# FofanovLab/mtsv_tools

Measured on NVIDIA B200. Metric: reads/sec binned (150 bp), higher is better.
Workload: dtype u8/u32 integer

## Files before the change

### mtsv_tools_b200/csrc/binner.cu

```cuda
#include <algorithm>
#include <thread>

#include "ctx.h"

#ifndef MTSV_COALESCE_UNROLL
#define MTSV_COALESCE_UNROLL 4
#endif
#ifndef MTSV_COALESCE_TILES
#define MTSV_COALESCE_TILES 4
#endif
constexpr int kCoalesceTiles = MTSV_COALESCE_TILES;
constexpr int kCoalesceUnroll = MTSV_COALESCE_UNROLL;

namespace mtsv {

constexpr uint32_t kMaxReadLenDev = MTSVGPU_MAX_READ_LEN;

__device__ __forceinline__ void cta_accumulate(unsigned long long* counters32, unsigned int v) {
  __shared__ unsigned int cta_sum;
  if (threadIdx.x == 0) cta_sum = 0;
  __syncthreads();
  unsigned int w = __reduce_add_sync(0xffffffffu, v);
  if ((threadIdx.x & 31) == 0 && w) atomicAdd(&cta_sum, w);
  __syncthreads();
// ... 232 lines not shown
    unsigned big = __ballot_sync(0xffffffffu, cnt > kSolo);
    while (big) {
      int src = __ffs(big) - 1;
      big &= big - 1;
      uint32_t c = __shfl_sync(0xffffffffu, cnt, src);
      uint32_t l = __shfl_sync(0xffffffffu, lo, src);
      uint32_t d = __shfl_sync(0xffffffffu, dst, src);
      for (uint32_t r = lane; r < c; r += 32)
        hit_keys[d + r] = make_hit_key(fm_locate(fm, sv, l + r, nullptr), qoff);
    }
  }
}

constexpr uint32_t kSortMedium = 4096;
constexpr uint32_t kLightItems = 16;
constexpr uint32_t kMonsterHits = 1024;

__device__ __forceinline__ uint64_t warp_sort_u64(uint64_t v, unsigned lane) {
#pragma unroll
  for (int k = 2; k <= 32; k <<= 1) {
    {
      uint64_t o = __shfl_xor_sync(0xffffffffu, v, k - 1);
      bool low = (lane & (k - 1)) < ((lane ^ (k - 1)) & (k - 1));
      v = low ? (v < o ? v : o) : (v > o ? v : o);
    }
#pragma unroll
    for (int j = k >> 2; j > 0; j >>= 1) {
      uint64_t o = __shfl_xor_sync(0xffffffffu, v, j);
      bool low = (lane & j) == 0;
      v = low ? (v < o ? v : o) : (v > o ? v : o);
    }
  }
  return v;
}

__global__ void __launch_bounds__(256) sort_classify_kernel(const uint32_t* __restrict__ seg_cnt, uint32_t nq,
                                                            uint32_t min_count, uint32_t* __restrict__ warp_list,
                                                            uint32_t* __restrict__ medium_list,
                                                            uint32_t* __restrict__ large_list,
                                                            BatchCounters* __restrict__ ctr) {
  uint32_t q = blockIdx.x * blockDim.x + threadIdx.x;
  const unsigned lane = threadIdx.x & 31;
  uint32_t n = q < nq ? seg_cnt[q] : 0;
  int cls = n <= min_count || n < 2 ? -1 : (n <= 32 ? 0 : (n <= kSortMedium ? 1 : 2));
#pragma unroll
  for (int c = 0; c < 3; ++c) {
    unsigned m = __ballot_sync(0xffffffffu, cls == c);
    if (!m) continue;
    unsigned int* counter = c == 0 ? &ctr->n_warp : (c == 1 ? &ctr->n_medium : &ctr->n_large);
    uint32_t* list = c == 0 ? warp_list : (c == 1 ? medium_list : large_list);
    uint32_t base = 0;
    if (lane == (unsigned)(__ffs(m) - 1)) base = atomicAdd(counter, (unsigned)__popc(m));
    base = __shfl_sync(0xffffffffu, base, __ffs(m) - 1);
    if (cls == c) list[base + __popc(m & ((1u << lane) - 1))] = q;
  }
}

__global__ void __launch_bounds__(256) sort_warp_kernel(uint64_t* __restrict__ keys,
                                                        const uint32_t* __restrict__ seg_off,
                                                        const uint32_t* __restrict__ seg_cnt,
                                                        const uint32_t* __restrict__ list,
                                                        const BatchCounters* __restrict__ ctr) {
  const unsigned lane = threadIdx.x & 31;
  const uint32_t n_list = ctr->n_warp;
  const uint32_t warps = (gridDim.x * blockDim.x) >> 5;
  for (uint32_t it = (blockIdx.x * blockDim.x + threadIdx.x) >> 5; it < n_list; it += warps) {
    uint32_t q = list[it];
    uint32_t n = seg_cnt[q];
    uint64_t* base = keys + seg_off[q];
    uint64_t v = lane < n ? base[lane] : ~0ull;
// ... 100 lines not shown
  CE(0, 1) CE(2, 3) CE(4, 5) CE(6, 7) CE(8, 9) CE(10, 11) CE(12, 13) CE(14, 15)
  CE(0, 2) CE(1, 3) CE(4, 6) CE(5, 7) CE(8, 10) CE(9, 11) CE(12, 14) CE(13, 15)
  CE(1, 2) CE(5, 6) CE(9, 10) CE(13, 14) CE(0, 4) CE(1, 5) CE(2, 6) CE(3, 7)
  CE(8, 12) CE(9, 13) CE(10, 14) CE(11, 15) CE(2, 4) CE(3, 5) CE(10, 12) CE(11, 13)
  CE(1, 2) CE(3, 4) CE(5, 6) CE(9, 10) CE(11, 12) CE(13, 14) CE(0, 8) CE(1, 9)
  CE(2, 10) CE(3, 11) CE(4, 12) CE(5, 13) CE(6, 14) CE(7, 15) CE(4, 8) CE(5, 9)
  CE(6, 10) CE(7, 11) CE(2, 4) CE(3, 5) CE(6, 8) CE(7, 9) CE(10, 12) CE(11, 13)
  CE(1, 2) CE(3, 4) CE(5, 6) CE(7, 8) CE(9, 10) CE(11, 12) CE(13, 14)
#undef CE
}

__device__ __forceinline__ bool carry_valid_or_lane(unsigned lane, bool carry_valid) {
  return lane > 0 || carry_valid;
}

__device__ uint32_t coalesce_warp(const BinsView& bv, const uint64_t* __restrict__ keys, uint32_t n_hits,
                                  uint32_t min_seeds, uint32_t L, uint32_t k, CandRec* __restrict__ cand) {
  const unsigned lane = threadIdx.x & 31;
  uint32_t nc = 0;
  bool have = false;
  CandRec cur{0, 0, 0, 0};
  uint32_t carry_site = 0, carry_bin = 0;
  bool carry_valid = false;
  constexpr int U = kCoalesceTiles;
  uint32_t top = 1;
  while (top < bv.n) top <<= 1;
  for (uint32_t g0 = 0; g0 < n_hits; g0 += 32 * U) {
    uint32_t site[U], qoff[U], b[U], ws[U], we[U];
    bool some[U];
#pragma unroll
    for (int u = 0; u < U; ++u) {
      uint32_t h = g0 + u * 32 + lane;
      uint64_t key = h < n_hits ? keys[h] : 0;
      site[u] = (uint32_t)(key >> 16);
      qoff[u] = (uint32_t)(key & 0xffff);
      b[u] = 0;
    }
    for (uint32_t step = top; step >= 1; step >>= 1) {
#pragma unroll
// ... 75 lines not shown
          have = some_i;
          if (some_i) cur = CandRec{ws_i, we_i, b_i, 1};
        }
      }
    }
  }
  if (have && cur.num_seeds >= min_seeds) {
    if (lane == 0) {
      cand[nc] = cur;
    }
    ++nc;
  }
  return nc;
}

__global__ void __launch_bounds__(128) coalesce_kernel(BinsView bv, ReadsView rv, Params p, uint32_t nq,
                                                       const uint32_t* __restrict__ hit_off,
                                                       const uint32_t* __restrict__ q_nhits,
                                                       const uint32_t* __restrict__ q_nseeds,
                                                       uint64_t* __restrict__ hit_keys,
                                                       CandRec* __restrict__ cand_sparse,
                                                       uint32_t* __restrict__ q_ncand,
                                                       uint32_t* __restrict__ heavy_list,
                                                       uint32_t* __restrict__ monster_list,
                                                       BatchCounters* __restrict__ ctr) {
  const uint32_t r = blockIdx.x * blockDim.x + threadIdx.x;
  const unsigned lane = threadIdx.x & 31;
  uint32_t first = 0;
  if (p.ns == 2 && r * 2 + 1 < nq && q_nhits[r * 2 + 1] > q_nhits[r * 2]) first = 1;
  for (uint32_t pass = 0; pass < p.ns; ++pass) {
    const uint32_t s = p.ns == 2 ? (pass ^ first) : 0;
    const uint32_t q = r * p.ns + s;
    uint32_t nh = q < nq ? q_nhits[q] : 0;
    if (pass == 1 && !__any_sync(0xffffffffu, nh != 0)) {
      if (q < nq) q_ncand[q] = 0;
      continue;
    }
    uint32_t nc = 0, L = 0, k = 0, ms = 0, base = 0;
    if (nh) {
      L = query_len(rv, p.ns, q);
      k = edit_budget(L, p.edit_rate);
      ms = min_seeds_of(q_nseeds[q], p.min_seed);
      base = hit_off[q];
      if (nh <= kLightItems) {
        uint64_t* kq = hit_keys + base;
        if (nh > 1) {
          uint64_t v[kLightItems];
#pragma unroll
          for (uint32_t i = 0; i < kLightItems; ++i) v[i] = i < nh ? kq[i] : ~0ull;
          static_assert(kLightItems == 16, "sort_network16 sorts exactly 16 keys");
          sort_network16(v);
#pragma unroll
          for (uint32_t i = 0; i < kLightItems; ++i)
            if (i < nh) kq[i] = v[i];
        }
        nc = coalesce_item(bv, kq, nh, ms, L, k, cand_sparse + base);
      }
    }
    unsigned heavy = __ballot_sync(0xffffffffu, nh > kLightItems && nh <= kMonsterHits);
    if (heavy) {
      uint32_t slot = 0;
      if (lane == (unsigned)(__ffs(heavy) - 1)) slot = atomicAdd(&ctr->n_heavy, (unsigned)__popc(heavy));
      slot = __shfl_sync(0xffffffffu, slot, __ffs(heavy) - 1);
      if (nh > kLightItems && nh <= kMonsterHits) heavy_list[slot + __popc(heavy & ((1u << lane) - 1))] = q;
    }
    if (nh > kMonsterHits) monster_list[atomicAdd(&ctr->n_monster, 1u)] = q;
    if (q < nq && nh <= kLightItems) q_ncand[q] = nc;
  }
}

__global__ void __launch_bounds__(128) coalesce_heavy_kernel(BinsView bv, ReadsView rv, Params p,
                                                             const uint32_t* __restrict__ hit_off,
                                                             const uint32_t* __restrict__ q_nhits,
                                                             const uint32_t* __restrict__ q_nseeds,
                                                             const uint64_t* __restrict__ hit_keys,
                                                             CandRec* __restrict__ cand_sparse,
                                                             uint32_t* __restrict__ q_ncand,
                                                             const uint32_t* __restrict__ heavy_list,
                                                             BatchCounters* __restrict__ ctr) {
  const unsigned lane = threadIdx.x & 31;
  const uint32_t n_list = ctr->n_heavy;
  for (;;) {
// ... 63 lines not shown
      uint32_t run = 0;
      for (int i = 0; i < 32; ++i) {
        s_pre[i] = run;
        run += s_cnt[i];
      }
      s_pre[32] = run;
      q_ncand[q] = run;
    }
    __syncthreads();
    for (uint32_t i = lane; i < cnt; i += 32) cand_sparse[base + s_pre[w] + i] = cand_stage[base + my_start + i];
    __syncthreads();
  }
}

__global__ void __launch_bounds__(256) rank_emit_kernel(uint32_t nq, const uint32_t* __restrict__ hit_off,
                                                        const uint32_t* __restrict__ q_ncand,
                                                        const uint32_t* __restrict__ cand_off,
                                                        const CandRec* __restrict__ cand_sparse,
                                                        CandRec* __restrict__ cand_dense,
                                                        uint32_t* __restrict__ cand_q) {
  uint32_t q = blockIdx.x * blockDim.x + threadIdx.x;
  const unsigned lane = threadIdx.x & 31;
  uint32_t nc = q < nq ? q_ncand[q] : 0;
  uint32_t src = 0, dst = 0;
  if (nc) {
    src = hit_off[q];
    dst = cand_off[q];
    if (nc <= kLightItems) {
      uint64_t prev = 0;
      for (uint32_t i = 0; i < nc; ++i) {
        uint64_t best = ~0ull;
        for (uint32_t j = 0; j < nc; ++j) {
          uint64_t kj = make_rank_key(cand_sparse[src + j].num_seeds, j);
          if ((i == 0 || kj > prev) && kj < best) best = kj;
        }
        prev = best;
        cand_dense[dst + i] = cand_sparse[src + (uint32_t)(best & 0xffffffffu)];
        cand_q[dst + i] = q;
      }
    }
  }
  unsigned heavy = __ballot_sync(0xffffffffu, nc > kLightItems);
  while (heavy) {
    int sl = __ffs(heavy) - 1;
    heavy &= heavy - 1;
    const uint32_t nc_s = __shfl_sync(0xffffffffu, nc, sl), src_s = __shfl_sync(0xffffffffu, src, sl);
    const uint32_t dst_s = __shfl_sync(0xffffffffu, dst, sl), q_s = __shfl_sync(0xffffffffu, q, sl);
    uint32_t out = 0;
    uint32_t bound = 0xffffffffu;
    while (out < nc_s) {
      uint32_t v = 0;
      for (uint32_t i = lane; i < nc_s; i += 32) {
        uint32_t ns = cand_sparse[src_s + i].num_seeds;
        if (ns < bound && ns > v) v = ns;
      }
      v = __reduce_max_sync(0xffffffffu, v);
      for (uint32_t t0 = 0; t0 < nc_s; t0 += 32) {
// ... 625 lines not shown
    return set_error(MTSVGPU_EINVAL, "seed_size must be in [1,4096]");
  if (in->seed_gap == 0)
    return set_error(MTSVGPU_EINVAL, "seed_gap must be > 0");
  p->edit_rate = in->edit_rate;
  p->min_seed = in->min_seed;
  p->S = in->seed_size;
  p->G = in->seed_gap;
  p->max_hits = in->max_hits;
  p->tune_max_hits = in->tune_max_hits;
  p->max_candidates = in->max_candidates < 0 ? -1 : in->max_candidates;
  p->max_assignments = in->max_assignments < 0 ? -1 : in->max_assignments;
  p->ns = in->strands == 1 ? 1 : 2;
  return 0;
}

int run_segmented_sort(cudaStream_t st, DevBuf& worklist, uint64_t* keys, const uint32_t* seg_off,
                              const uint32_t* seg_cnt, uint32_t nq, uint32_t min_count, BatchCounters* d_ctr) {
  if (worklist.cap < (size_t)3 * nq * 4) {
    MTSV_CUDA_TRY(cudaStreamSynchronize(st));
    MTSV_TRY(worklist.reserve((size_t)3 * nq * 4));
  }
  uint32_t* lists = worklist.as<uint32_t>();
  MTSV_CUDA_TRY(cudaMemsetAsync(&d_ctr->n_warp, 0, 3 * sizeof(unsigned int), st));
  MTSV_LAUNCH(sort_classify_kernel, (nq + 255) / 256, 256, 0, st, seg_cnt, nq, min_count, lists, lists + nq,
              lists + 2 * (size_t)nq, d_ctr);
  MTSV_LAUNCH(sort_warp_kernel, sm_count() * 8, 256, 0, st, keys, seg_off, seg_cnt, lists, d_ctr);
  MTSV_LAUNCH(sort_medium_kernel, sm_count() * 4, 512, 0, st, keys, seg_off, seg_cnt, lists + nq, d_ctr);
  MTSV_LAUNCH(sort_large_kernel, sm_count(), 1024, 0, st, keys, seg_off, seg_cnt, lists + 2 * (size_t)nq, d_ctr);
  MTSV_CUDA_TRY(cudaGetLastError());
  return 0;
}

static int grow_preserve(DevBuf& buf, size_t used_bytes, size_t need_bytes, cudaStream_t st) {
  if (need_bytes <= buf.cap && buf.p) return 0;
  size_t want = std::max(need_bytes + need_bytes / 2, (size_t)1 << 20);
  DevPtr<uint8_t> np;
  MTSV_TRY(dev_alloc(np, want));
  if (buf.p && used_bytes) {
    MTSV_CUDA_TRY(cudaMemcpyAsync(np.get(), buf.p.get(), used_bytes, cudaMemcpyDeviceToDevice, st));
    MTSV_CUDA_TRY(cudaStreamSynchronize(st));
  }
  buf.p = std::move(np);
  buf.cap = want;
// ... 201 lines not shown
    if (rv.n_reads == 1)
      return set_error(MTSVGPU_ELIMIT, "one read produced %llu seed hits (cap %llu)", hc.total_hits,
                       (unsigned long long)hit_cap);
    return 1;
  }
  n_hits = (uint32_t)hc.total_hits;
  ln.stats.n_seed_hits += n_hits;
  for (int i = 0; i < 32; ++i) ln.stats.rank_queries += hc.rank_steps[i];
  return 0;
}

int SubBatch::candidates() {
  const DeviceIndex& ix = h->ix;
  for (DevBuf* b : {&ws.q_ncand, &ws.cand_off}) MTSV_TRY(b->reserve(qn * 4));
  if (!n_hits) return 0;
  MTSV_TRY(ws.worklist.reserve(3 * qn * 4));
  MTSV_TRY(ws.hit_keys.reserve((size_t)n_hits * 8));
  MTSV_TRY(ws.cand_sparse.reserve((size_t)n_hits * sizeof(CandRec)));
  begin(ST_LOCATE);
  MTSV_LAUNCH(locate_kernel, qgrid(), 256, 0, st, ix.fm_view(), ix.sa_view(), p, ws.slot_off.as<uint32_t>(), nq,
              ws.slot_lo.as<uint32_t>(), ws.slot_cnt.as<uint32_t>(), ws.slot_hoff.as<uint32_t>(),
              ws.hit_off.as<uint32_t>(), ws.q_nhits.as<uint32_t>(), ws.hit_keys.as<uint64_t>());
  end();
  begin(ST_SORT);
  MTSV_TRY(run_segmented_sort(st, ws.worklist, ws.hit_keys.as<uint64_t>(), ws.hit_off.as<uint32_t>(),
                              ws.q_nhits.as<uint32_t>(), nq, kLightItems, d_ctr));
  end();
  begin(ST_COALESCE);
  MTSV_TRY(ws.cand_stage.reserve((size_t)n_hits * sizeof(CandRec)));
  MTSV_CUDA_TRY(cudaMemsetAsync(&d_ctr->n_heavy, 0, 3 * sizeof(unsigned int), st));
  MTSV_LAUNCH(coalesce_kernel, (rv.n_reads + 127) / 128, 128, 0, st, ix.bins_view(), rv, p, nq,
              ws.hit_off.as<uint32_t>(), ws.q_nhits.as<uint32_t>(), ws.q_nseeds.as<uint32_t>(),
              ws.hit_keys.as<uint64_t>(), ws.cand_sparse.as<CandRec>(), ws.q_ncand.as<uint32_t>(),
              ws.worklist.as<uint32_t>(), ws.worklist.as<uint32_t>() + nq, d_ctr);
  MTSV_LAUNCH(coalesce_heavy_kernel, sm_count() * 16, 128, 0, st, ix.bins_view(), rv, p, ws.hit_off.as<uint32_t>(),
              ws.q_nhits.as<uint32_t>(), ws.q_nseeds.as<uint32_t>(), ws.hit_keys.as<uint64_t>(),
              ws.cand_sparse.as<CandRec>(), ws.q_ncand.as<uint32_t>(), ws.worklist.as<uint32_t>(), d_ctr);
  MTSV_LAUNCH(coalesce_monster_kernel, sm_count(), 1024, 0, st, ix.bins_view(), rv, p, ws.hit_off.as<uint32_t>(),
              ws.q_nhits.as<uint32_t>(), ws.q_nseeds.as<uint32_t>(), ws.hit_keys.as<uint64_t>(),
              ws.cand_sparse.as<CandRec>(), ws.cand_stage.as<CandRec>(), ws.q_ncand.as<uint32_t>(),
              ws.worklist.as<uint32_t>() + nq, d_ctr);
  MTSV_TRY(exclusive_scan_u32(ws.q_ncand.as<uint32_t>(), ws.cand_off.as<uint32_t>(), nq, ws.scan_tmp,
                              (uint64_t*)&d_ctr->total_cands, st));
  end();
  MTSV_TRY(fetch());
  n_cand = (uint32_t)hc.total_cands;
  if (!n_cand) return 0;
  MTSV_TRY(ws.cand_dense.reserve((size_t)n_cand * sizeof(CandRec)));
  MTSV_TRY(ws.cand_q.reserve((size_t)n_cand * 4));
  begin(ST_RANK);
  MTSV_LAUNCH(rank_emit_kernel, qgrid(), 256, 0, st, nq, ws.hit_off.as<uint32_t>(), ws.q_ncand.as<uint32_t>(),
              ws.cand_off.as<uint32_t>(), ws.cand_sparse.as<CandRec>(), ws.cand_dense.as<CandRec>(),
              ws.cand_q.as<uint32_t>());
  end();
  return 0;
}

int SubBatch::verify() {
  const bool ssw = hc.max_len >= 254;
  bool grouped = !ssw && (group_verify ? group_verify[0] != '0' : n_cand > nq && h->ix.n_bins > h->ix.n_taxids);
  MTSV_TRY(ws.cand_edit.reserve((size_t)n_cand * 4));
  begin(ST_VERIFY);
  MTSV_TRY(ws.cand_flag.reserve(((size_t)n_cand + 1) * 4));
  MTSV_TRY(ws.cand_order.reserve((size_t)n_cand * 4));
  MTSV_LAUNCH(cand_class_kernel, (n_cand + 255) / 256, 256, 0, st, ws.cand_dense.as<CandRec>(), n_cand,
              ws.cand_flag.as<uint32_t>(), (h->profiling && !grouped) ? d_ctr : nullptr, 1);
  MTSV_TRY(exclusive_scan_u32(ws.cand_flag.as<uint32_t>(), ws.cand_flag.as<uint32_t>(), n_cand, ws.scan_tmp,
                              nullptr, st));
// ... 79 lines not shown
  if (n2) {
    MTSV_LAUNCH(cand_compact_order_kernel, grid, 256, 0, st, ws.cand_order.as<uint32_t>(), flag, n_cand,
                ws.cand_dense.as<CandRec>(), ws.cand_order2.as<uint32_t>(), ctr);
    round_jobs.n = n2;
    MTSV_TRY(launch_verify_warp(round_jobs));
  }
  n_verified = (uint64_t)n1 + n2;
  return 0;
}

int SubBatch::merge_taxids() {
  const uint32_t nr = rv.n_reads;
  uint64_t* keys = ws.hit_keys.as<uint64_t>();
  MTSV_LAUNCH(taxid_keys_kernel, (nq + 1 + 255) / 256, 256, 0, st, nq, p.ns, ws.cand_off.as<uint32_t>(),
              ws.out_off.as<uint32_t>(), ws.hit_tmp.as<HitRec>(), keys, seg_off(), seg_cnt());
  MTSV_TRY(run_segmented_sort(st, ws.worklist, keys, seg_off(), seg_cnt(), nr, 1, d_ctr));
  MTSV_LAUNCH(taxid_count_kernel, (nr + 255) / 256, 256, 0, st, keys, seg_off(), nr, tax_cnt());
  MTSV_TRY(exclusive_scan_u32(tax_cnt(), tax_off(), nr, ws.scan_tmp, (uint64_t*)&d_ctr->total_taxhits, st));
  return 0;
}

int SubBatch::select_append(uint64_t* out_total) {
  for (DevBuf* b : {&ws.q_nout, &ws.out_off}) MTSV_TRY(b->reserve(qn * 4));
  const bool taxhits = kind == BatchOutput::TaxHits;
  uint64_t sub_out = 0, sub_tax = 0;
  if (n_cand) {
    MTSV_TRY(ws.hit_tmp.reserve((size_t)n_cand * sizeof(HitRec)));
    begin(ST_EMIT);
    MTSV_LAUNCH(select_kernel, (nq + 127) / 128, 128, 0, st, h->ix.bins_view(), rv, p, nq, ws.cand_off.as<uint32_t>(),
                ws.cand_dense.as<CandRec>(), ws.cand_edit.as<uint32_t>(), ws.hit_tmp.as<HitRec>(),
                ws.q_nout.as<uint32_t>());
// ... 313 lines not shown
```

### mtsv_tools_b200/csrc/collapse.cu

```cuda
#include <mutex>

#include "ctx.h"

namespace mtsv {

struct PartsView {
  const mtsvgpu_hit* hits[16];
  const uint32_t* counts[16];
  const uint32_t* offs[16];
  uint32_t n_parts;
};

__global__ void collapse_total_kernel(PartsView pv, uint32_t n_reads, uint32_t* __restrict__ total) {
  uint32_t r = blockIdx.x * blockDim.x + threadIdx.x;
  if (r >= n_reads) return;
  uint32_t t = 0;
  for (uint32_t p = 0; p < pv.n_parts; ++p) t += pv.counts[p][r];
  total[r] = t;
}

__global__ void collapse_scatter_kernel(PartsView pv, uint32_t n_reads, const uint32_t* __restrict__ comb_off,
                                        uint64_t* __restrict__ keys) {
  uint32_t t = blockIdx.x * blockDim.x + threadIdx.x;
  uint32_t r = t / pv.n_parts, p = t % pv.n_parts;
// ... 122 lines not shown
  MTSV_TRY(cnt_out.reserve(((size_t)nr + 1) * 4));
  MTSV_TRY(off_out32.reserve(((size_t)nr + 1) * 4));
  const unsigned rgrid = (nr + 255) / 256 + 1;
  if (nr) MTSV_LAUNCH(collapse_total_kernel, rgrid, 256, 0, st, pv, nr, total.as<uint32_t>());
  MTSV_TRY(exclusive_scan_u32(total.as<uint32_t>(), comb_off.as<uint32_t>(), nr, scan_tmp, d_tot, st));
  uint64_t h_tot = 0;
  MTSV_CUDA_TRY(cudaMemcpyAsync(&h_tot, d_tot, 8, cudaMemcpyDeviceToHost, st));
  MTSV_CUDA_TRY(cudaStreamSynchronize(st));
  if (h_tot > 0xfffffff0ull) return set_error(MTSVGPU_ELIMIT, "more than 2^32 hits in one collapse call");
  MTSV_TRY(keys.reserve((size_t)(h_tot + 1) * 8));
  if (nr && h_tot) {
    const uint64_t threads = (uint64_t)nr * n_parts;
    MTSV_LAUNCH(collapse_scatter_kernel, (unsigned)((threads + 255) / 256), 256, 0, st, pv, nr,
                comb_off.as<uint32_t>(), keys.as<uint64_t>());
    MTSV_TRY(run_segmented_sort(st, worklist, keys.as<uint64_t>(), comb_off.as<uint32_t>(), total.as<uint32_t>(), nr,
                                1, counters.as<BatchCounters>()));
  }
  if (nr) MTSV_LAUNCH(collapse_count_kernel, rgrid, 256, 0, st, keys.as<uint64_t>(), comb_off.as<uint32_t>(), nr,
                      cnt_out.as<uint32_t>());
  MTSV_TRY(exclusive_scan_u32(cnt_out.as<uint32_t>(), off_out32.as<uint32_t>(), nr, scan_tmp, d_tot, st));
  MTSV_CUDA_TRY(cudaMemcpyAsync(&h_tot, d_tot, 8, cudaMemcpyDeviceToHost, st));
  MTSV_CUDA_TRY(cudaStreamSynchronize(st));
  DevPtr<mtsvgpu_taxhit> out;
  DevPtr<uint64_t> out_off;
  MTSV_TRY(dev_alloc(out, h_tot + 1));
  MTSV_TRY(dev_alloc(out_off, (uint64_t)nr + 1));
  MTSV_LAUNCH(collapse_write_kernel, rgrid, 256, 0, st, keys.as<uint64_t>(), comb_off.as<uint32_t>(),
              off_out32.as<uint32_t>(), nr, out.get(), out_off.get());
  cudaError_t e = cudaStreamSynchronize(st);
  if (e != cudaSuccess) return set_error(MTSVGPU_ECUDA, "collapse: %s", cudaGetErrorString(e));
  *d_out = out.release();
// ... 22 lines not shown
    pv.offs[p] = w.offs[p].as<uint32_t>();
  }
  MTSV_TRY(w.total.reserve(((size_t)nr + 1) * 4));
  MTSV_TRY(w.comb_off.reserve(((size_t)nr + 1) * 4));
  MTSV_TRY(w.cnt_out.reserve(((size_t)nr + 1) * 4));
  MTSV_TRY(w.off_out32.reserve(((size_t)nr + 1) * 4));
  MTSV_TRY(w.keys.reserve((size_t)(hit_cap + 1) * 8));
  const unsigned rgrid = (nr + 255) / 256 + 1;
  if (nr) MTSV_LAUNCH(collapse_total_kernel, rgrid, 256, 0, st, pv, nr, w.total.as<uint32_t>());
  MTSV_TRY(exclusive_scan_u32(w.total.as<uint32_t>(), w.comb_off.as<uint32_t>(), nr, w.scan_tmp, d_tot, st));
  if (nr) {
    const uint64_t threads = (uint64_t)nr * n_parts;
    MTSV_LAUNCH(collapse_scatter_kernel, (unsigned)((threads + 255) / 256), 256, 0, st, pv, nr,
                w.comb_off.as<uint32_t>(), w.keys.as<uint64_t>());
    MTSV_TRY(run_segmented_sort(st, w.worklist, w.keys.as<uint64_t>(), w.comb_off.as<uint32_t>(), w.total.as<uint32_t>(),
                                nr, 1, w.counters.as<BatchCounters>()));
    MTSV_LAUNCH(collapse_count_kernel, rgrid, 256, 0, st, w.keys.as<uint64_t>(), w.comb_off.as<uint32_t>(), nr,
                w.cnt_out.as<uint32_t>());
  }
  MTSV_TRY(exclusive_scan_u32(w.cnt_out.as<uint32_t>(), w.off_out32.as<uint32_t>(), nr, w.scan_tmp, d_n_out, st));
  MTSV_LAUNCH(collapse_write_kernel, rgrid, 256, 0, st, w.keys.as<uint64_t>(), w.comb_off.as<uint32_t>(),
              w.off_out32.as<uint32_t>(), nr, out, out_off);
  MTSV_CUDA_TRY(cudaGetLastError());
  return 0;
}

int collapse_device_long(int device, cudaStream_t st, uint32_t n_parts, const mtsvgpu_hit* const* d_hits,
                         const uint32_t* const* d_counts, uint64_t n_reads, mtsvgpu_hit** d_out,
                         uint64_t** d_out_off, uint64_t* n_out) {
  if (!d_hits || !d_counts || !d_out || !d_out_off || !n_out) return set_error(MTSVGPU_EINVAL, "null argument");
  if (n_parts == 0 || n_parts > 16) return set_error(MTSVGPU_EINVAL, "n_parts must be in [1,16]");
// ... 58 lines not shown
```

### mtsv_tools_b200/csrc/core.cuh

```cuda
#pragma once
#include <stdint.h>

#include <algorithm>
#include <vector>

#if defined(__CUDACC__)
#define MTSV_HD __host__ __device__ __forceinline__
#else
#define MTSV_HD inline
struct uint2 {
  uint32_t x, y;
};
#endif

namespace mtsv {

MTSV_HD int popc64(uint64_t x) {
#ifdef __CUDA_ARCH__
  return __popcll(x);
#else
  return __builtin_popcountll(x);
#endif
}

// ... 505 lines not shown
  double v = (double)n_seeds * pct;
  double f = (double)(int64_t)v;
  if (f < 1.0) f = 1.0;
  if (f > 4294967295.0) f = 4294967295.0;
  return (uint32_t)f;
}

struct CandRec {
  uint32_t start, end, bin, num_seeds;
};

MTSV_HD uint64_t make_rank_key(uint32_t num_seeds, uint32_t idx) {
  return ((uint64_t)(~num_seeds) << 32) | idx;
}

MTSV_HD uint32_t coalesce_item(const BinsView& bv, const uint64_t* keys, uint32_t n_hits,
                               uint32_t min_seeds, uint32_t L, uint32_t k, CandRec* cand) {
  uint32_t nc = 0;
  bool have = false;
  CandRec cur{0, 0, 0, 0};
  uint32_t b = 0, b_start = 0, b_end = 0;
  bool b_valid = false;
  for (uint32_t h = 0; h < n_hits; ++h) {
    uint64_t key = keys[h];
    uint32_t site = (uint32_t)(key >> 16), q_off = (uint32_t)(key & 0xffff);
    if (!b_valid || site >= b_end) {
      b = find_bin(bv, site);
      b_start = ldg(&bv.start[b]);
      b_end = ldg(&bv.end[b]);
      b_valid = true;
    }
    uint32_t ws = 0, we = 0;
    bool some = candidate_window(site, q_off, b_start, b_end, L, k, &ws, &we);
    bool merged = false;
    if (have && some && b == cur.bin &&
        ((cur.start <= ws && ws < cur.end) || (cur.start < we && we <= cur.end))) {
      cur.start = ws < cur.start ? ws : cur.start;
      cur.end = we > cur.end ? we : cur.end;
      cur.num_seeds += 1;
      merged = true;
    }
    if (!merged) {
      if (have && cur.num_seeds >= min_seeds) {
        cand[nc] = cur;
        ++nc;
      }
      have = some;
      if (some) cur = CandRec{ws, we, b, 1};
    }
  }
  if (have && cur.num_seeds >= min_seeds) {
    cand[nc] = cur;
    ++nc;
  }
  return nc;
}

constexpr uint32_t kNoEdit = 0xffffffffu;

MTSV_HD void myers_block(uint64_t Eq, uint64_t& Pv, uint64_t& Mv, uint32_t& phin, uint32_t& mhin,
                         uint64_t& Ph_out, uint64_t& Mh_out) {
  uint64_t Xv = Eq | Mv;
  Eq |= (uint64_t)mhin;
  uint64_t Xh = (((Eq & Pv) + Pv) ^ Pv) | Eq;
  uint64_t Ph = Mv | ~(Xh | Pv);
  uint64_t Mh = Pv & Xh;
  Ph_out = Ph;
  Mh_out = Mh;
// ... 431 lines not shown
```

### mtsv_tools_b200/csrc/ctx.h

```cpp
#pragma once
#include <cuda_runtime.h>
#include <stdarg.h>
#include <stdint.h>

#include <algorithm>
#include <atomic>
#include <condition_variable>
#include <memory>
#include <mutex>
#include <string>
#include <vector>

#include "../../include/mtsv_b200.h"
#include "core.cuh"

namespace mtsv {

int set_error(int code, const char* fmt, ...);
unsigned sm_count();
extern std::atomic<uint64_t> g_launches;

#define MTSV_CUDA_TRY(expr)                                                                  \
  do {                                                                                       \
    cudaError_t e_ = (expr);                                                                 \
// ... 220 lines not shown
                int device, const mtsvgpu_index_opts* opts, mtsvgpu_index** out);
int index_write(mtsvgpu_index* h, const char* path, uint32_t sample_interval, uint32_t sa_sample);
int index_export(mtsvgpu_index* h, uint8_t* text_out, uint8_t* bwt_out, uint64_t* sample_out, uint32_t sa_sample);
int suffix_array_host(int device, const uint8_t* text, uint64_t n, uint32_t* sa_out, uint8_t* bwt_out);
int bin_batch_device(mtsvgpu_index* h, const uint8_t* d_seqs, const uint64_t* d_seq_off,
                     uint64_t n_reads, BatchSource* src, BatchOutput kind,
                     const mtsvgpu_params* params, const void** d_out,
                     const uint64_t** d_out_off, uint64_t* n_out);
int backward_search_batch(mtsvgpu_index* h, const uint8_t* pats, uint32_t pat_len, uint64_t n_pats,
                          uint64_t* lower, uint64_t* upper);
int locate_batch(mtsvgpu_index* h, const uint64_t* rows, uint64_t n_rows, uint64_t* pos);
int edit_distance_batch(int device, const uint8_t* pats, const uint64_t* pat_off,
                        const uint8_t* texts, const uint64_t* text_off, uint64_t n_pairs,
                        uint32_t* edits);
int run_segmented_sort(cudaStream_t st, DevBuf& worklist, uint64_t* keys, const uint32_t* seg_off,
                       const uint32_t* seg_cnt, uint32_t nq, uint32_t min_count, BatchCounters* d_ctr);
int collapse_device(int device, cudaStream_t st, uint32_t n_parts, const mtsvgpu_hit* const* d_hits,
                    const uint32_t* const* d_counts, uint64_t n_reads, mtsvgpu_taxhit** d_out,
                    uint64_t** d_out_off, uint64_t* n_out);
int collapse_device_long(int device, cudaStream_t st, uint32_t n_parts, const mtsvgpu_hit* const* d_hits,
                         const uint32_t* const* d_counts, uint64_t n_reads, mtsvgpu_hit** d_out,
                         uint64_t** d_out_off, uint64_t* n_out);
struct CollapseScratch {
  DevBuf offs[16], total, comb_off, keys, scan_tmp, counters, worklist, cnt_out, off_out32;
};
int collapse_taxid_async(CollapseScratch& w, cudaStream_t st, uint32_t n_parts, const mtsvgpu_hit* const* d_hits,
                         const uint32_t* const* d_counts, uint32_t nr, uint64_t hit_cap, mtsvgpu_taxhit* out,
                         uint64_t* out_off, uint64_t* d_n_out);
int comm_create(int device, uint32_t rank, uint32_t world, uint64_t max_local_reads, uint64_t max_hits_per_source,
                mtsvgpu_comm** out, uint8_t* handle_out);
int comm_connect(mtsvgpu_comm* c, const uint8_t* all_handles);
// ... 8 lines not shown
```

Baseline: 490.3 million.

## Fuse small-segment sorting and candidate ranking into the coalesce kernel

Removes the separate segmented-sort pass ahead of coalescing. Reads with up to 16 hits are sorted in registers and ranked by seed count in-thread. Reads with 17–32 hits are warp-sorted, coalesced and ranked inside the coalesce kernel, and the medium/large sort lists are built there too, so the sort kernels only handle big segments afterwards. rank_emit then does a warp-cooperative copy for pre-ranked reads instead of an O(n²) selection per thread. This saves launches and global round-trips of the hit keys, but adds register pressure and warp-serial work to the coalesce kernel.

```diff
diff --git a/mtsv_tools_b200/csrc/binner.cu b/mtsv_tools_b200/csrc/binner.cu
--- a/mtsv_tools_b200/csrc/binner.cu
+++ b/mtsv_tools_b200/csrc/binner.cu
@@ -270,6 +270,7 @@
 
 constexpr uint32_t kSortMedium = 4096;
 constexpr uint32_t kLightItems = 16;
+constexpr uint32_t kWarpHits = 32;
 constexpr uint32_t kMonsterHits = 1024;
 
 __device__ __forceinline__ uint64_t warp_sort_u64(uint64_t v, unsigned lane) {
@@ -290,26 +291,26 @@
   return v;
 }
 
+__device__ __forceinline__ void warp_append(uint32_t* __restrict__ list, unsigned int* counter, bool pred, uint32_t q) {
+  const unsigned lane = threadIdx.x & 31;
+  const unsigned m = __ballot_sync(0xffffffffu, pred);
+  if (!m) return;
+  uint32_t base = 0;
+  if (lane == (unsigned)(__ffs(m) - 1)) base = atomicAdd(counter, (unsigned)__popc(m));
+  base = __shfl_sync(0xffffffffu, base, __ffs(m) - 1);
+  if (pred) list[base + __popc(m & ((1u << lane) - 1))] = q;
+}
+
 __global__ void __launch_bounds__(256) sort_classify_kernel(const uint32_t* __restrict__ seg_cnt, uint32_t nq,
-                                                            uint32_t min_count, uint32_t* __restrict__ warp_list,
+                                                            uint32_t* __restrict__ warp_list,
                                                             uint32_t* __restrict__ medium_list,
                                                             uint32_t* __restrict__ large_list,
                                                             BatchCounters* __restrict__ ctr) {
   uint32_t q = blockIdx.x * blockDim.x + threadIdx.x;
-  const unsigned lane = threadIdx.x & 31;
   uint32_t n = q < nq ? seg_cnt[q] : 0;
-  int cls = n <= min_count || n < 2 ? -1 : (n <= 32 ? 0 : (n <= kSortMedium ? 1 : 2));
-#pragma unroll
-  for (int c = 0; c < 3; ++c) {
-    unsigned m = __ballot_sync(0xffffffffu, cls == c);
-    if (!m) continue;
-    unsigned int* counter = c == 0 ? &ctr->n_warp : (c == 1 ? &ctr->n_medium : &ctr->n_large);
-    uint32_t* list = c == 0 ? warp_list : (c == 1 ? medium_list : large_list);
-    uint32_t base = 0;
-    if (lane == (unsigned)(__ffs(m) - 1)) base = atomicAdd(counter, (unsigned)__popc(m));
-    base = __shfl_sync(0xffffffffu, base, __ffs(m) - 1);
-    if (cls == c) list[base + __popc(m & ((1u << lane) - 1))] = q;
-  }
+  warp_append(warp_list, &ctr->n_warp, n >= 2 && n <= 32, q);
+  warp_append(medium_list, &ctr->n_medium, n > 32 && n <= kSortMedium, q);
+  warp_append(large_list, &ctr->n_large, n > kSortMedium, q);
 }
 
 __global__ void __launch_bounds__(256) sort_warp_kernel(uint64_t* __restrict__ keys,
@@ -440,6 +441,7 @@
   return lane > 0 || carry_valid;
 }
 
+template <int U = kCoalesceTiles>
 __device__ uint32_t coalesce_warp(const BinsView& bv, const uint64_t* __restrict__ keys, uint32_t n_hits,
                                   uint32_t min_seeds, uint32_t L, uint32_t k, CandRec* __restrict__ cand) {
   const unsigned lane = threadIdx.x & 31;
@@ -448,7 +450,6 @@
   CandRec cur{0, 0, 0, 0};
   uint32_t carry_site = 0, carry_bin = 0;
   bool carry_valid = false;
-  constexpr int U = kCoalesceTiles;
   uint32_t top = 1;
   while (top < bv.n) top <<= 1;
   for (uint32_t g0 = 0; g0 < n_hits; g0 += 32 * U) {
@@ -554,15 +555,21 @@
   return nc;
 }
 
+struct HeavyLists {
+  uint32_t* sort_medium;
+  uint32_t* sort_large;
+  uint32_t* heavy;
+  uint32_t* monster;
+};
+
 __global__ void __launch_bounds__(128) coalesce_kernel(BinsView bv, ReadsView rv, Params p, uint32_t nq,
                                                        const uint32_t* __restrict__ hit_off,
                                                        const uint32_t* __restrict__ q_nhits,
                                                        const uint32_t* __restrict__ q_nseeds,
                                                        uint64_t* __restrict__ hit_keys,
                                                        CandRec* __restrict__ cand_sparse,
-                                                       uint32_t* __restrict__ q_ncand,
-                                                       uint32_t* __restrict__ heavy_list,
-                                                       uint32_t* __restrict__ monster_list,
+                                                       CandRec* __restrict__ cand_stage,
+                                                       uint32_t* __restrict__ q_ncand, HeavyLists lists,
                                                        BatchCounters* __restrict__ ctr) {
   const uint32_t r = blockIdx.x * blockDim.x + threadIdx.x;
   const unsigned lane = threadIdx.x & 31;
@@ -571,7 +578,7 @@
   for (uint32_t pass = 0; pass < p.ns; ++pass) {
     const uint32_t s = p.ns == 2 ? (pass ^ first) : 0;
     const uint32_t q = r * p.ns + s;
-    uint32_t nh = q < nq ? q_nhits[q] : 0;
+    const uint32_t nh = q < nq ? q_nhits[q] : 0;
     if (pass == 1 && !__any_sync(0xffffffffu, nh != 0)) {
       if (q < nq) q_ncand[q] = 0;
       continue;
@@ -582,30 +589,47 @@
       k = edit_budget(L, p.edit_rate);
       ms = min_seeds_of(q_nseeds[q], p.min_seed);
       base = hit_off[q];
-      if (nh <= kLightItems) {
-        uint64_t* kq = hit_keys + base;
-        if (nh > 1) {
-          uint64_t v[kLightItems];
+      if (nh <= kLightHits) {
+        const uint64_t* kq = hit_keys + base;
+        uint64_t v[kLightHits];
 #pragma unroll
-          for (uint32_t i = 0; i < kLightItems; ++i) v[i] = i < nh ? kq[i] : ~0ull;
-          static_assert(kLightItems == 16, "sort_network16 sorts exactly 16 keys");
-          sort_network16(v);
-#pragma unroll
-          for (uint32_t i = 0; i < kLightItems; ++i)
-            if (i < nh) kq[i] = v[i];
-        }
-        nc = coalesce_item(bv, kq, nh, ms, L, k, cand_sparse + base);
-      }
-    }
-    unsigned heavy = __ballot_sync(0xffffffffu, nh > kLightItems && nh <= kMonsterHits);
-    if (heavy) {
-      uint32_t slot = 0;
-      if (lane == (unsigned)(__ffs(heavy) - 1)) slot = atomicAdd(&ctr->n_heavy, (unsigned)__popc(heavy));
-      slot = __shfl_sync(0xffffffffu, slot, __ffs(heavy) - 1);
-      if (nh > kLightItems && nh <= kMonsterHits) heavy_list[slot + __popc(heavy & ((1u << lane) - 1))] = q;
-    }
-    if (nh > kMonsterHits) monster_list[atomicAdd(&ctr->n_monster, 1u)] = q;
-    if (q < nq && nh <= kLightItems) q_ncand[q] = nc;
+        for (uint32_t i = 0; i < kLightHits; ++i) v[i] = i < nh ? kq[i] : ~0ull;
+        static_assert(kLightHits == 16, "sort_network16 sorts exactly 16 keys");
+        if (nh > 1) sort_network16(v);
+        nc = coalesce_light(bv, v, nh, ms, L, k, cand_sparse + base, cand_stage + base);
+      }
+    }
+    if (q < nq && nh <= kLightHits) q_ncand[q] = nc;
+
+    unsigned todo = __ballot_sync(0xffffffffu, nh > kLightHits && nh <= kWarpHits);
+    while (todo) {
+      const int src = __ffs(todo) - 1;
+      todo &= todo - 1;
+      const uint32_t n = __shfl_sync(0xffffffffu, nh, src), bs = __shfl_sync(0xffffffffu, base, src);
+      const uint32_t qs = __shfl_sync(0xffffffffu, q, src);
+      uint64_t key = lane < n ? hit_keys[bs + lane] : ~0ull;
+      key = warp_sort_u64(key, lane);
+      if (lane < n) hit_keys[bs + lane] = key;
+      __syncwarp();
+      const uint32_t ncw = coalesce_warp<1>(bv, hit_keys + bs, n, __shfl_sync(0xffffffffu, ms, src),
+                                            __shfl_sync(0xffffffffu, L, src), __shfl_sync(0xffffffffu, k, src),
+                                            cand_stage + bs);
+      __syncwarp();
+      CandRec c{0, 0, 0, 0};
+      if (lane < ncw) c = cand_stage[bs + lane];
+      uint32_t rk = 0;
+      for (uint32_t i = 0; i < ncw; ++i) {
+        const uint32_t sd = __shfl_sync(0xffffffffu, c.num_seeds, i);
+        rk += (sd > c.num_seeds || (i < lane && sd == c.num_seeds)) ? 1u : 0u;
+      }
+      if (lane < ncw) cand_sparse[bs + rk] = c;
+      if (lane == 0) q_ncand[qs] = ncw;
+    }
+
+    warp_append(lists.sort_medium, &ctr->n_medium, nh > kWarpHits && nh <= kSortMedium, q);
+    warp_append(lists.sort_large, &ctr->n_large, nh > kSortMedium, q);
+    warp_append(lists.heavy, &ctr->n_heavy, nh > kWarpHits && nh <= kMonsterHits, q);
+    warp_append(lists.monster, &ctr->n_monster, nh > kMonsterHits, q);
   }
 }
 
@@ -699,6 +723,7 @@
 }
 
 __global__ void __launch_bounds__(256) rank_emit_kernel(uint32_t nq, const uint32_t* __restrict__ hit_off,
+                                                        const uint32_t* __restrict__ q_nhits,
                                                         const uint32_t* __restrict__ q_ncand,
                                                         const uint32_t* __restrict__ cand_off,
                                                         const CandRec* __restrict__ cand_sparse,
@@ -708,24 +733,35 @@
   const unsigned lane = threadIdx.x & 31;
   uint32_t nc = q < nq ? q_ncand[q] : 0;
   uint32_t src = 0, dst = 0;
+  bool ranked = false;
   if (nc) {
     src = hit_off[q];
     dst = cand_off[q];
-    if (nc <= kLightItems) {
-      uint64_t prev = 0;
-      for (uint32_t i = 0; i < nc; ++i) {
-        uint64_t best = ~0ull;
-        for (uint32_t j = 0; j < nc; ++j) {
-          uint64_t kj = make_rank_key(cand_sparse[src + j].num_seeds, j);
-          if ((i == 0 || kj > prev) && kj < best) best = kj;
-        }
-        prev = best;
-        cand_dense[dst + i] = cand_sparse[src + (uint32_t)(best & 0xffffffffu)];
-        cand_q[dst + i] = q;
-      }
-    }
-  }
-  unsigned heavy = __ballot_sync(0xffffffffu, nc > kLightItems);
+    ranked = q_nhits[q] <= kWarpHits;
+  }
+  const uint32_t n_copy = ranked ? nc : 0;
+  uint32_t incl = n_copy;
+#pragma unroll
+  for (uint32_t d = 1; d < 32; d <<= 1) {
+    const uint32_t t = __shfl_up_sync(0xffffffffu, incl, d);
+    if (lane >= d) incl += t;
+  }
+  const uint32_t total = __shfl_sync(0xffffffffu, incl, 31);
+  for (uint32_t t0 = 0; t0 < total; t0 += 32) {
+    const uint32_t t = t0 + lane;
+    uint32_t j = 0;
+#pragma unroll
+    for (uint32_t step = 16; step; step >>= 1)
+      if (__shfl_sync(0xffffffffu, incl, j + step - 1) <= t) j += step;
+    const uint32_t e = t - (__shfl_sync(0xffffffffu, incl, j) - __shfl_sync(0xffffffffu, n_copy, j));
+    const uint32_t s_j = __shfl_sync(0xffffffffu, src, j), d_j = __shfl_sync(0xffffffffu, dst, j);
+    const uint32_t q_j = __shfl_sync(0xffffffffu, q, j);
+    if (t < total) {
+      cand_dense[d_j + e] = cand_sparse[s_j + e];
+      cand_q[d_j + e] = q_j;
+    }
+  }
+  unsigned heavy = __ballot_sync(0xffffffffu, nc != 0 && !ranked);
   while (heavy) {
     int sl = __ffs(heavy) - 1;
     heavy &= heavy - 1;
@@ -1381,19 +1417,25 @@
   return 0;
 }
 
+static int sort_listed(cudaStream_t st, uint64_t* keys, const uint32_t* seg_off, const uint32_t* seg_cnt,
+                       const uint32_t* medium_list, const uint32_t* large_list, BatchCounters* d_ctr) {
+  MTSV_LAUNCH(sort_medium_kernel, sm_count() * 4, 512, 0, st, keys, seg_off, seg_cnt, medium_list, d_ctr);
+  MTSV_LAUNCH(sort_large_kernel, sm_count(), 1024, 0, st, keys, seg_off, seg_cnt, large_list, d_ctr);
+  return 0;
+}
+
 int run_segmented_sort(cudaStream_t st, DevBuf& worklist, uint64_t* keys, const uint32_t* seg_off,
-                              const uint32_t* seg_cnt, uint32_t nq, uint32_t min_count, BatchCounters* d_ctr) {
+                       const uint32_t* seg_cnt, uint32_t nq, BatchCounters* d_ctr) {
   if (worklist.cap < (size_t)3 * nq * 4) {
     MTSV_CUDA_TRY(cudaStreamSynchronize(st));
     MTSV_TRY(worklist.reserve((size_t)3 * nq * 4));
   }
   uint32_t* lists = worklist.as<uint32_t>();
   MTSV_CUDA_TRY(cudaMemsetAsync(&d_ctr->n_warp, 0, 3 * sizeof(unsigned int), st));
-  MTSV_LAUNCH(sort_classify_kernel, (nq + 255) / 256, 256, 0, st, seg_cnt, nq, min_count, lists, lists + nq,
+  MTSV_LAUNCH(sort_classify_kernel, (nq + 255) / 256, 256, 0, st, seg_cnt, nq, lists, lists + nq,
               lists + 2 * (size_t)nq, d_ctr);
   MTSV_LAUNCH(sort_warp_kernel, sm_count() * 8, 256, 0, st, keys, seg_off, seg_cnt, lists, d_ctr);
-  MTSV_LAUNCH(sort_medium_kernel, sm_count() * 4, 512, 0, st, keys, seg_off, seg_cnt, lists + nq, d_ctr);
-  MTSV_LAUNCH(sort_large_kernel, sm_count(), 1024, 0, st, keys, seg_off, seg_cnt, lists + 2 * (size_t)nq, d_ctr);
+  MTSV_TRY(sort_listed(st, keys, seg_off, seg_cnt, lists + nq, lists + 2 * (size_t)nq, d_ctr));
   MTSV_CUDA_TRY(cudaGetLastError());
   return 0;
 }
@@ -1625,32 +1667,37 @@
   const DeviceIndex& ix = h->ix;
   for (DevBuf* b : {&ws.q_ncand, &ws.cand_off}) MTSV_TRY(b->reserve(qn * 4));
   if (!n_hits) return 0;
-  MTSV_TRY(ws.worklist.reserve(3 * qn * 4));
+  MTSV_TRY(ws.worklist.reserve(4 * qn * 4));
   MTSV_TRY(ws.hit_keys.reserve((size_t)n_hits * 8));
   MTSV_TRY(ws.cand_sparse.reserve((size_t)n_hits * sizeof(CandRec)));
+  MTSV_TRY(ws.cand_stage.reserve((size_t)n_hits * sizeof(CandRec)));
+  uint32_t* wl = ws.worklist.as<uint32_t>();
+  const HeavyLists lists{wl, wl + nq, wl + 2 * (size_t)nq, wl + 3 * (size_t)nq};
   begin(ST_LOCATE);
   MTSV_LAUNCH(locate_kernel, qgrid(), 256, 0, st, ix.fm_view(), ix.sa_view(), p, ws.slot_off.as<uint32_t>(), nq,
               ws.slot_lo.as<uint32_t>(), ws.slot_cnt.as<uint32_t>(), ws.slot_hoff.as<uint32_t>(),
               ws.hit_off.as<uint32_t>(), ws.q_nhits.as<uint32_t>(), ws.hit_keys.as<uint64_t>());
   end();
-  begin(ST_SORT);
-  MTSV_TRY(run_segmented_sort(st, ws.worklist, ws.hit_keys.as<uint64_t>(), ws.hit_off.as<uint32_t>(),
-                              ws.q_nhits.as<uint32_t>(), nq, kLightItems, d_ctr));
-  end();
   begin(ST_COALESCE);
-  MTSV_TRY(ws.cand_stage.reserve((size_t)n_hits * sizeof(CandRec)));
+  MTSV_CUDA_TRY(cudaMemsetAsync(&d_ctr->n_warp, 0, 3 * sizeof(unsigned int), st));
   MTSV_CUDA_TRY(cudaMemsetAsync(&d_ctr->n_heavy, 0, 3 * sizeof(unsigned int), st));
   MTSV_LAUNCH(coalesce_kernel, (rv.n_reads + 127) / 128, 128, 0, st, ix.bins_view(), rv, p, nq,
               ws.hit_off.as<uint32_t>(), ws.q_nhits.as<uint32_t>(), ws.q_nseeds.as<uint32_t>(),
-              ws.hit_keys.as<uint64_t>(), ws.cand_sparse.as<CandRec>(), ws.q_ncand.as<uint32_t>(),
-              ws.worklist.as<uint32_t>(), ws.worklist.as<uint32_t>() + nq, d_ctr);
+              ws.hit_keys.as<uint64_t>(), ws.cand_sparse.as<CandRec>(), ws.cand_stage.as<CandRec>(),
+              ws.q_ncand.as<uint32_t>(), lists, d_ctr);
+  end();
+  begin(ST_SORT);
+  MTSV_TRY(sort_listed(st, ws.hit_keys.as<uint64_t>(), ws.hit_off.as<uint32_t>(), ws.q_nhits.as<uint32_t>(),
+                       lists.sort_medium, lists.sort_large, d_ctr));
+  end();
+  begin(ST_COALESCE);
   MTSV_LAUNCH(coalesce_heavy_kernel, sm_count() * 16, 128, 0, st, ix.bins_view(), rv, p, ws.hit_off.as<uint32_t>(),
               ws.q_nhits.as<uint32_t>(), ws.q_nseeds.as<uint32_t>(), ws.hit_keys.as<uint64_t>(),
-              ws.cand_sparse.as<CandRec>(), ws.q_ncand.as<uint32_t>(), ws.worklist.as<uint32_t>(), d_ctr);
+              ws.cand_sparse.as<CandRec>(), ws.q_ncand.as<uint32_t>(), lists.heavy, d_ctr);
   MTSV_LAUNCH(coalesce_monster_kernel, sm_count(), 1024, 0, st, ix.bins_view(), rv, p, ws.hit_off.as<uint32_t>(),
               ws.q_nhits.as<uint32_t>(), ws.q_nseeds.as<uint32_t>(), ws.hit_keys.as<uint64_t>(),
               ws.cand_sparse.as<CandRec>(), ws.cand_stage.as<CandRec>(), ws.q_ncand.as<uint32_t>(),
-              ws.worklist.as<uint32_t>() + nq, d_ctr);
+              lists.monster, d_ctr);
   MTSV_TRY(exclusive_scan_u32(ws.q_ncand.as<uint32_t>(), ws.cand_off.as<uint32_t>(), nq, ws.scan_tmp,
                               (uint64_t*)&d_ctr->total_cands, st));
   end();
@@ -1660,9 +1707,9 @@
   MTSV_TRY(ws.cand_dense.reserve((size_t)n_cand * sizeof(CandRec)));
   MTSV_TRY(ws.cand_q.reserve((size_t)n_cand * 4));
   begin(ST_RANK);
-  MTSV_LAUNCH(rank_emit_kernel, qgrid(), 256, 0, st, nq, ws.hit_off.as<uint32_t>(), ws.q_ncand.as<uint32_t>(),
-              ws.cand_off.as<uint32_t>(), ws.cand_sparse.as<CandRec>(), ws.cand_dense.as<CandRec>(),
-              ws.cand_q.as<uint32_t>());
+  MTSV_LAUNCH(rank_emit_kernel, qgrid(), 256, 0, st, nq, ws.hit_off.as<uint32_t>(), ws.q_nhits.as<uint32_t>(),
+              ws.q_ncand.as<uint32_t>(), ws.cand_off.as<uint32_t>(), ws.cand_sparse.as<CandRec>(),
+              ws.cand_dense.as<CandRec>(), ws.cand_q.as<uint32_t>());
   end();
   return 0;
 }
@@ -1772,7 +1819,7 @@
   uint64_t* keys = ws.hit_keys.as<uint64_t>();
   MTSV_LAUNCH(taxid_keys_kernel, (nq + 1 + 255) / 256, 256, 0, st, nq, p.ns, ws.cand_off.as<uint32_t>(),
               ws.out_off.as<uint32_t>(), ws.hit_tmp.as<HitRec>(), keys, seg_off(), seg_cnt());
-  MTSV_TRY(run_segmented_sort(st, ws.worklist, keys, seg_off(), seg_cnt(), nr, 1, d_ctr));
+  MTSV_TRY(run_segmented_sort(st, ws.worklist, keys, seg_off(), seg_cnt(), nr, d_ctr));
   MTSV_LAUNCH(taxid_count_kernel, (nr + 255) / 256, 256, 0, st, keys, seg_off(), nr, tax_cnt());
   MTSV_TRY(exclusive_scan_u32(tax_cnt(), tax_off(), nr, ws.scan_tmp, (uint64_t*)&d_ctr->total_taxhits, st));
   return 0;
diff --git a/mtsv_tools_b200/csrc/collapse.cu b/mtsv_tools_b200/csrc/collapse.cu
--- a/mtsv_tools_b200/csrc/collapse.cu
+++ b/mtsv_tools_b200/csrc/collapse.cu
@@ -160,7 +160,7 @@
     MTSV_LAUNCH(collapse_scatter_kernel, (unsigned)((threads + 255) / 256), 256, 0, st, pv, nr,
                 comb_off.as<uint32_t>(), keys.as<uint64_t>());
     MTSV_TRY(run_segmented_sort(st, worklist, keys.as<uint64_t>(), comb_off.as<uint32_t>(), total.as<uint32_t>(), nr,
-                                1, counters.as<BatchCounters>()));
+                                counters.as<BatchCounters>()));
   }
   if (nr) MTSV_LAUNCH(collapse_count_kernel, rgrid, 256, 0, st, keys.as<uint64_t>(), comb_off.as<uint32_t>(), nr,
                       cnt_out.as<uint32_t>());
@@ -213,7 +213,7 @@
     MTSV_LAUNCH(collapse_scatter_kernel, (unsigned)((threads + 255) / 256), 256, 0, st, pv, nr,
                 w.comb_off.as<uint32_t>(), w.keys.as<uint64_t>());
     MTSV_TRY(run_segmented_sort(st, w.worklist, w.keys.as<uint64_t>(), w.comb_off.as<uint32_t>(), w.total.as<uint32_t>(),
-                                nr, 1, w.counters.as<BatchCounters>()));
+                                nr, w.counters.as<BatchCounters>()));
     MTSV_LAUNCH(collapse_count_kernel, rgrid, 256, 0, st, w.keys.as<uint64_t>(), w.comb_off.as<uint32_t>(), nr,
                 w.cnt_out.as<uint32_t>());
   }
diff --git a/mtsv_tools_b200/csrc/core.cuh b/mtsv_tools_b200/csrc/core.cuh
--- a/mtsv_tools_b200/csrc/core.cuh
+++ b/mtsv_tools_b200/csrc/core.cuh
@@ -543,15 +543,16 @@
   return ((uint64_t)(~num_seeds) << 32) | idx;
 }
 
-MTSV_HD uint32_t coalesce_item(const BinsView& bv, const uint64_t* keys, uint32_t n_hits,
-                               uint32_t min_seeds, uint32_t L, uint32_t k, CandRec* cand) {
-  uint32_t nc = 0;
+struct Coalescer {
+  const BinsView& bv;
+  uint32_t min_seeds, L, k;
   bool have = false;
   CandRec cur{0, 0, 0, 0};
   uint32_t b = 0, b_start = 0, b_end = 0;
   bool b_valid = false;
-  for (uint32_t h = 0; h < n_hits; ++h) {
-    uint64_t key = keys[h];
+
+  template <class Emit>
+  MTSV_HD void push(uint64_t key, Emit&& emit) {
     uint32_t site = (uint32_t)(key >> 16), q_off = (uint32_t)(key & 0xffff);
     if (!b_valid || site >= b_end) {
       b = find_bin(bv, site);
@@ -561,26 +562,76 @@
     }
     uint32_t ws = 0, we = 0;
     bool some = candidate_window(site, q_off, b_start, b_end, L, k, &ws, &we);
-    bool merged = false;
     if (have && some && b == cur.bin &&
         ((cur.start <= ws && ws < cur.end) || (cur.start < we && we <= cur.end))) {
       cur.start = ws < cur.start ? ws : cur.start;
       cur.end = we > cur.end ? we : cur.end;
       cur.num_seeds += 1;
-      merged = true;
-    }
-    if (!merged) {
-      if (have && cur.num_seeds >= min_seeds) {
-        cand[nc] = cur;
-        ++nc;
-      }
-      have = some;
-      if (some) cur = CandRec{ws, we, b, 1};
-    }
-  }
-  if (have && cur.num_seeds >= min_seeds) {
-    cand[nc] = cur;
+      return;
+    }
+    if (have && cur.num_seeds >= min_seeds) emit(cur);
+    have = some;
+    if (some) cur = CandRec{ws, we, b, 1};
+  }
+  template <class Emit>
+  MTSV_HD void finish(Emit&& emit) {
+    if (have && cur.num_seeds >= min_seeds) emit(cur);
+  }
+};
+
+MTSV_HD uint32_t coalesce_item(const BinsView& bv, const uint64_t* keys, uint32_t n_hits,
+                               uint32_t min_seeds, uint32_t L, uint32_t k, CandRec* cand) {
+  uint32_t nc = 0;
+  auto emit = [&](const CandRec& c) { cand[nc++] = c; };
+  Coalescer co{bv, min_seeds, L, k};
+  for (uint32_t h = 0; h < n_hits; ++h) co.push(keys[h], emit);
+  co.finish(emit);
+  return nc;
+}
+
+constexpr uint32_t kLightHits = 16;
+
+MTSV_HD uint64_t bytes_above(uint64_t x, uint32_t s) {
+  return (x + 0x0101010101010101ull * (uint64_t)(0x7fu - s)) & 0x8080808080808080ull;
+}
+
+MTSV_HD uint32_t light_rank(uint64_t lo, uint64_t hi, uint32_t i, uint32_t s) {
+  const uint64_t glo = bytes_above(lo, s), ghi = bytes_above(hi, s);
+  const uint64_t elo = bytes_above(lo, s - 1) & ~glo, ehi = bytes_above(hi, s - 1) & ~ghi;
+  const uint64_t before_lo = i >= 8 ? ~0ull : (1ull << (8 * i)) - 1;
+  const uint64_t before_hi = i <= 8 ? 0ull : (1ull << (8 * (i - 8))) - 1;
+  return (uint32_t)(popc64(glo) + popc64(ghi) + popc64(elo & before_lo) + popc64(ehi & before_hi));
+}
+
+MTSV_HD uint32_t coalesce_light(const BinsView& bv, uint64_t (&v)[kLightHits], uint32_t n_hits, uint32_t min_seeds,
+                                uint32_t L, uint32_t k, CandRec* out, CandRec* stage) {
+  uint32_t nc = 0, prev = ~0u;
+  uint64_t ns_lo = 0, ns_hi = 0;
+  bool ranked = true;
+  auto emit = [&](const CandRec& c) {
+    out[nc] = c;
+    if (nc < 8) ns_lo |= (uint64_t)c.num_seeds << (8 * nc);
+    else ns_hi |= (uint64_t)c.num_seeds << (8 * (nc - 8));
+    ranked = ranked && c.num_seeds <= prev;
+    prev = c.num_seeds;
     ++nc;
+  };
+  Coalescer co{bv, min_seeds, L, k};
+  for (uint32_t h = 0; h < n_hits; ++h) {
+    const uint64_t x = v[0];
+#ifdef __CUDA_ARCH__
+#pragma unroll
+#endif
+    for (uint32_t i = 0; i + 1 < kLightHits; ++i) v[i] = v[i + 1];
+    co.push(x, emit);
+  }
+  co.finish(emit);
+  if (!ranked) {
+    for (uint32_t i = 0; i < nc; ++i) {
+      const uint64_t w = i < 8 ? ns_lo : ns_hi;
+      stage[light_rank(ns_lo, ns_hi, i, (uint32_t)(w >> (8 * (i & 7))) & 0xff)] = out[i];
+    }
+    for (uint32_t i = 0; i < nc; ++i) out[i] = stage[i];
   }
   return nc;
 }
diff --git a/mtsv_tools_b200/csrc/ctx.h b/mtsv_tools_b200/csrc/ctx.h
--- a/mtsv_tools_b200/csrc/ctx.h
+++ b/mtsv_tools_b200/csrc/ctx.h
@@ -258,7 +258,7 @@
                         const uint8_t* texts, const uint64_t* text_off, uint64_t n_pairs,
                         uint32_t* edits);
 int run_segmented_sort(cudaStream_t st, DevBuf& worklist, uint64_t* keys, const uint32_t* seg_off,
-                       const uint32_t* seg_cnt, uint32_t nq, uint32_t min_count, BatchCounters* d_ctr);
+                       const uint32_t* seg_cnt, uint32_t nq, BatchCounters* d_ctr);
 int collapse_device(int device, cudaStream_t st, uint32_t n_parts, const mtsvgpu_hit* const* d_hits,
                     const uint32_t* const* d_counts, uint64_t n_reads, mtsvgpu_taxhit** d_out,
                     uint64_t** d_out_off, uint64_t* n_out);
```

Result: no change. 492.6 million (median of 6 runs) (+0.5%).
